# Maryamsana-1998/DiffCodec-Controlling-Latent-Diffusion-for-Perceptual-Video-Compression

Hardware: AMD Instinct MI355X
Metric: decoded frames/sec @ 512x512, 20-step DDIM, GOP-12 (higher is better)
Workload: dtype bf16; 1 GPU; 512x512 inter frames of a GOP-12 clip, 16 per step per GPU, 20-step DDIM, CFG 4.5 (model batch 32), control scale 1.7, SD-1.5 + DualFlowControlNet + VAE decode, random-init weights; hip_graphs=True, parallelism=unit-shard x1, backend=none, backend_world_size=1

## Files before the change

diffcodec-controlling-latent-diffusion-for-perceptual-video-compression_amd/csrc/attention.hip:

```cpp
#include "dc_common.h"
#include "../../include/diffcodec_hip.h"
#include <cstdlib>
#include <type_traits>

#ifdef DC_STAMP
__device__ unsigned long long dc_attn_stamp_buf[1 << 18];
extern "C" int dc_attn_stamp_read(void* dst, int n) { return (int)hipMemcpyFromSymbol(dst, HIP_SYMBOL(dc_attn_stamp_buf), (size_t)n * 8); }
#define DC_NOW(t) asm volatile("s_memtime %0\n\ts_waitcnt lgkmcnt(0)" : "=s"(t)::"memory")
#define DC_NOW_RT(t) asm volatile("s_memrealtime %0\n\ts_waitcnt lgkmcnt(0)" : "=s"(t)::"memory")
#define DC_STAMP_SLOTS 16
#else
#define DC_NOW(t) (void)0
#define DC_NOW_RT(t) (void)0
#endif

namespace {

constexpr int KV_TILE = 64;
constexpr float RESCALE_THR = 4.0f;
typedef __attribute__((ext_vector_type(4))) short s16x4;
typedef __attribute__((address_space(3))) s16x4* lds_s16x4_ptr;
__host__ __device__ constexpr int v_pitch_bytes(int ndt) { return ndt * 64 <= 64 ? 64 : (ndt * 64 <= 192 ? 192 : 320); }

struct AttnArgs {
    const bf16_t* q;
    const bf16_t* k;
    const bf16_t* v;
    bf16_t* o;
    int B, heads, Nq, Nk;
    long long qs, ks, vs, os;
    float scale_log2e;
    int xcd_remap;
};

constexpr int SHORT_PASSES = 4;
template <int D, int QB, bool SHORT, bool RAGGED, bool PP = false>
__global__ __launch_bounds__(PP ? 512 : 256, (D <= 80 ? 2 : 1)) void attn_kernel(const AttnArgs a)
{
    static_assert(!PP || !SHORT, "ping-pong is the long-context form");
    constexpr int NWAVE = PP ? 8 : 4, NT = NWAVE * 64;
    constexpr int ND16 = (D + 15) / 16;
    constexpr int NDT = (D + 31) / 32;
    constexpr int NV = D / 8;
    constexpr int KP16 = (ND16 * 2) | 1;
    constexpr int K_PITCH = KP16 * 16;
    constexpr int K_BYTES = KV_TILE * K_PITCH;
    constexpr int V_PITCH = v_pitch_bytes(NDT);
    constexpr int VT_BYTES = KV_TILE * V_PITCH;
    constexpr int BUF = K_BYTES + VT_BYTES;
    constexpr int QW = 32 * QB;
    constexpr int OPITCH = D * 2 + 16;
    static_assert(NDT <= 5, "head dim <= 160");
    constexpr bool QOFF = (D % 16) != 0 && !SHORT;
    constexpr int QOFF_KS = D / 16, QOFF_LH = (D % 16) / 8, QOFF_E = (D % 16) % 8;
    constexpr bool ONES = (D % 32) != 0;
    constexpr int ONES_T = D / 32, ONES_R = ((D % 32) & 3) + 4 * ((D % 32) >> 3);
    static_assert(!ONES || ((D % 32) % 8) < 4, "ones row must live in the lower lane half");
    constexpr int NLD = (KV_TILE * NV + 255) / 256;
    extern __shared__ __attribute__((aligned(16))) char smem[];

    const int tid = threadIdx.x, lane = tid & 63, wave = __builtin_amdgcn_readfirstlane(tid >> 6);
    const int lq = lane & 31, lh = lane >> 5;
    unsigned long long st_in = 0, rt_in = 0, rt_0 = 0, rt_e = 0, st_out = 0, rt_out = 0;
    DC_NOW(st_in);
    DC_NOW_RT(rt_in);
    constexpr int QWG = NWAVE * QW * (SHORT ? SHORT_PASSES : 1);
    const int qblocks = (a.Nq + QWG - 1) / QWG;
    int bid = blockIdx.x;
    if (a.xcd_remap) bid = dc_xcd_remap(bid, gridDim.x);
    const int bh = bid / qblocks;
    const int qb = bid - bh * qblocks;
    const int b = bh / a.heads, h = bh - b * a.heads;
    int q0 = qb * QWG + wave * QW;

    const bf16_t* __restrict__ Q = a.q + (long long)b * a.Nq * a.qs + h * D;
    const bf16_t* __restrict__ K = a.k + (long long)b * a.Nk * a.ks + h * D;
    const bf16_t* __restrict__ V = a.v + (long long)b * a.Nk * a.vs + h * D;

    for (int i = tid * 16; i < 2 * BUF; i += NT * 16) *(u32x4*)(smem + i) = u32x4{0u, 0u, 0u, 0u};
    if (ONES) {
        __syncthreads();
        if (tid < 2 * KV_TILE) {
            *(unsigned short*)(smem + (tid >> 6) * BUF + K_BYTES + (tid & 63) * V_PITCH + D * 2) = 0x3F80;
            if (QOFF) *(unsigned short*)(smem + (tid >> 6) * BUF + (tid & 63) * K_PITCH + D * 2) = 0x3F80;
        }
    }

    bf16x8 qf[QB][ND16];
    f32x16 oacc[QB][NDT];
    float m_run[QB], l_run[QB];
    auto fetch_q = [&](int qbase, bf16x8 (&dst)[QB][ND16]) {
#pragma unroll
        for (int u = 0; u < QB; ++u)
#pragma unroll
            for (int ks = 0; ks < ND16; ++ks) {
                const int dcol = 16 * ks + 8 * lh;
                const int qi = qbase + 32 * u + lq;
                u32x4 v = {0u, 0u, 0u, 0u};
                if (qi < a.Nq && dcol < D) v = *(const u32x4*)(Q + (long long)qi * a.qs + dcol);
                bf16x8 qv = *(bf16x8*)&v;
                if (QOFF) {
#pragma unroll
                    for (int e = 0; e < 8; ++e) qv[e] = (bf16_t)((float)qv[e] * a.scale_log2e);
                }
                dst[u][ks] = qv;
            }
    };
    auto reset_acc = [&]() {
#pragma unroll
        for (int u = 0; u < QB; ++u) {
#pragma unroll
            for (int t = 0; t < NDT; ++t)
#pragma unroll
                for (int r = 0; r < 16; ++r) oacc[u][t][r] = 0.f;
            m_run[u] = QOFF ? 0.f : -INFINITY;
            l_run[u] = 0.f;
        }
    };
    fetch_q(q0, qf);
    reset_acc();

    u32x4 rk[NLD], rv[NLD];
    const int ntiles = (a.Nk + KV_TILE - 1) / KV_TILE;

    constexpr int NVB = 4 * (NV / 4);
    auto v_piece = [&](int q, int& row, int& vec) {
        row = lane, vec = q;
        if (NVB > 0 && q < NVB) row = 16 * (q & 3) + (lane >> 2), vec = 4 * (q >> 2) + (lane & 3);
    };
    auto issue_loads = [&](int t) {
        const int kb = t * KV_TILE;
        int key = kb + lane;
        if (RAGGED) key = key < a.Nk ? key : a.Nk - 1;
#pragma unroll
        for (int i = 0; i < NLD; ++i) {
            const int vec = wave + 4 * i;
            if (vec < NV) {
                rk[i] = *(const u32x4*)(K + (long long)key * a.ks + vec * 8);
                int vrow, vvec;
                v_piece(vec, vrow, vvec);
                int vkey = kb + vrow;
                if (RAGGED) vkey = vkey < a.Nk ? vkey : a.Nk - 1;
                rv[i] = *(const u32x4*)(V + (long long)vkey * a.vs + vvec * 8);
            }
        }
    };
    auto store_lds = [&](int buf) {
        char* sK = smem + buf * BUF;
        char* sV = sK + K_BYTES;
#pragma unroll
        for (int i = 0; i < NLD; ++i) {
            const int vec = wave + 4 * i;
            if (vec < NV) {
                *(u32x4*)(sK + lane * K_PITCH + vec * 16) = rk[i];
                int vrow, vvec;
                v_piece(vec, vrow, vvec);
                *(u32x4*)(sV + vrow * V_PITCH + vvec * 16) = rv[i];
            }
        }
    };

    __syncthreads();
    if constexpr (!PP) {
        issue_loads(0);
        store_lds(0);
    }
    if constexpr (!PP) {
        __builtin_amdgcn_s_waitcnt(0x0F70);
        __syncthreads();
    }

    typedef __attribute__((ext_vector_type(2))) float f32x2;
    unsigned long long st_a = 0, st_b = 0, st_c = 0, st_d = 0, st_e = 0, s_qk = 0, s_sm = 0, s_pv = 0, s_st = 0, st_0 = 0, st_v = 0, s_vst = 0;
    DC_NOW(st_0);
    DC_NOW_RT(rt_0);
    f32x16 s[QB][2];
    bf16x8 pf[QB][2][2];
    int jn = 2;
    auto qk_part = [&](int buf) {
        const char* sK = smem + buf * BUF;
#pragma unroll
        for (int u = 0; u < QB; ++u)
#pragma unroll
            for (int j = 0; j < 2; ++j)
#pragma unroll
                for (int r = 0; r < 16; ++r) s[u][j][r] = 0.f;
#pragma unroll
        for (int j = 0; j < 2; ++j)
#pragma unroll
            for (int ks = 0; ks < ND16; ++ks) {
                if (j >= jn) continue;
                const bf16x8 kf = *(const bf16x8*)(sK + (32 * j + lq) * K_PITCH + (16 * ks + 8 * lh) * 2);
#pragma unroll
                for (int u = 0; u < QB; ++u) s[u][j] = __builtin_amdgcn_mfma_f32_32x32x16_bf16(kf, qf[u][ks], s[u][j], 0, 0, 0);
            }

    };
    float mloc_s[QB];
    auto rowmax_part = [&](int t) {
        const int kb = t * KV_TILE;
#pragma unroll
        for (int u = 0; u < QB; ++u) {
            if (RAGGED && kb + KV_TILE > a.Nk) {
#pragma unroll
                for (int j = 0; j < 2; ++j)
#pragma unroll
                    for (int r = 0; r < 16; ++r) {
                        if (j >= jn) continue;
                        const int key = kb + 32 * j + (r & 3) + 8 * (r >> 2) + 4 * lh;
                        if (key >= a.Nk) s[u][j][r] = -INFINITY;
                    }
            }
            float mloc = s[u][0][0];
#pragma unroll
            for (int j = 0; j < 2; ++j)
#pragma unroll
                for (int r = 0; r < 16; ++r)
                    if (j < jn) mloc = fmaxf(mloc, s[u][j][r]);
            {
                const auto sw = __builtin_amdgcn_permlane32_swap(__float_as_uint(mloc), __float_as_uint(mloc), false, false);
                mloc = fmaxf(__uint_as_float(sw[0]), __uint_as_float(sw[1]));
            }
            mloc_s[u] = mloc;
        }
    };
    auto softmax_part = [&](int t, bool first) {
        __builtin_amdgcn_s_setprio(2);
#pragma unroll
        for (int u = 0; u < QB; ++u) {
            const float mloc = mloc_s[u];
            if (QOFF) {
                const float m_next = (float)(bf16_t)(m_run[u] + mloc);
                const float delta = (first || mloc > RESCALE_THR) ? m_next - m_run[u] : 0.f;
                if (__any(delta != 0.f)) {
                    const float alpha = __builtin_amdgcn_exp2f(-delta);
#pragma unroll
                    for (int j = 0; j < 2; ++j)
#pragma unroll
                        for (int r = 0; r < 16; ++r) s[u][j][r] -= delta;
                    if (!ONES) l_run[u] *= alpha;
#pragma unroll
                    for (int tt = 0; tt < NDT; ++tt)
#pragma unroll
                        for (int r = 0; r < 16; ++r) oacc[u][tt][r] *= alpha;
                    m_run[u] += delta;
                    if (lh == QOFF_LH) qf[u][QOFF_KS][QOFF_E] = (bf16_t)(-m_run[u]);
                }
                float lsum = 0.f;
#pragma unroll
                for (int j = 0; j < 2; ++j)
#pragma unroll
                    for (int r = 0; r < 16; r += 2) {
                        const float p0 = __builtin_amdgcn_exp2f(s[u][j][r]), p1 = __builtin_amdgcn_exp2f(s[u][j][r + 1]);
                        if (!ONES) lsum += p0 + p1;
                        pf[u][j][r >> 3][r & 7] = (bf16_t)p0;
                        pf[u][j][r >> 3][(r & 7) + 1] = (bf16_t)p1;
                    }
                if (!ONES) l_run[u] += lsum;
                continue;
            }
            const float m_new = fmaxf(m_run[u], mloc);
            const float mc = m_new * a.scale_log2e;
            float lsum = 0.f;
#pragma unroll
            for (int j = 0; j < 2; ++j)
#pragma unroll
                for (int r = 0; r < 16; r += 2) {
                    if (j >= jn) continue;
                    const float t0 = __builtin_fmaf(s[u][j][r], a.scale_log2e, -mc), t1 = __builtin_fmaf(s[u][j][r + 1], a.scale_log2e, -mc);
                    const float p0 = __builtin_amdgcn_exp2f(t0), p1 = __builtin_amdgcn_exp2f(t1);
                    if (!ONES) lsum += p0 + p1;
                    pf[u][j][r >> 3][r & 7] = (bf16_t)p0;
                    pf[u][j][r >> 3][(r & 7) + 1] = (bf16_t)p1;
                }
            if (__any(m_new != m_run[u])) {
                const float alpha = __builtin_amdgcn_exp2f(m_run[u] * a.scale_log2e - mc);
                if (!ONES) l_run[u] *= alpha;
#pragma unroll
                for (int tt = 0; tt < NDT; ++tt)
#pragma unroll
                    for (int r = 0; r < 16; ++r) oacc[u][tt][r] *= alpha;
                m_run[u] = m_new;
            }
            if (!ONES) l_run[u] += lsum;
        }

        __builtin_amdgcn_s_setprio(0);
    };
    auto pv_part = [&](int buf) {
        const char* sV = smem + buf * BUF + K_BYTES;
        const char* vbase = sV + (4 * lh + ((lane & 15) >> 2)) * V_PITCH + (16 * ((lane >> 4) & 1) + 4 * (lane & 3)) * 2;
#pragma unroll
        for (int tt = 0; tt < NDT; ++tt) {
#pragma unroll
            for (int j = 0; j < 2; ++j)
#pragma unroll
                for (int s2 = 0; s2 < 2; ++s2) {
                    if (j >= jn) continue;
                    const char* pk = vbase + (32 * j + 16 * s2) * V_PITCH + tt * 64;
                    const s16x4 lo = __builtin_amdgcn_ds_read_tr16_b64_v4i16((lds_s16x4_ptr)pk);
                    const s16x4 hi = __builtin_amdgcn_ds_read_tr16_b64_v4i16((lds_s16x4_ptr)(pk + 8 * V_PITCH));
                    u32x2 l2 = *(const u32x2*)&lo, h2 = *(const u32x2*)&hi;
                    u32x4 av = {l2[0], l2[1], h2[0], h2[1]};
#pragma unroll
                    for (int u = 0; u < QB; ++u)
                        oacc[u][tt] = __builtin_amdgcn_mfma_f32_32x32x16_bf16(*(bf16x8*)&av, pf[u][j][s2], oacc[u][tt], 0, 0, 0);
                }
        }
    };
    auto process_tile = [&](int t, bool first, bool stage_next) {
        qk_part(t & 1);
        rowmax_part(t);
#ifdef DC_STAMP
        __builtin_amdgcn_sched_barrier(0);
        DC_NOW(st_b);
#endif
        softmax_part(t, first);
#ifdef DC_STAMP
        __builtin_amdgcn_sched_barrier(0);
        DC_NOW(st_c);
#endif
        if (stage_next) store_lds((t & 1) ^ 1);
        pv_part(t & 1);
    };

    auto store_out = [&]() {
#pragma unroll
    for (int u = 0; u < QB; ++u) {
        float l_tot;
        if (ONES) l_tot = __shfl(oacc[u][ONES_T][ONES_R], lq, 64);
        else l_tot = l_run[u] + __shfl_xor(l_run[u], 32, 64);
        const float inv = 1.0f / l_tot;
        const int qi = q0 + 32 * u + lq;
        if constexpr (SHORT) {
            char* stg = smem + 2 * BUF + wave * (QW * OPITCH) + (32 * u + lq) * OPITCH;
#pragma unroll
            for (int tt = 0; tt < NDT; ++tt)
#pragma unroll
                for (int g = 0; g < 4; ++g) {
                    const int dcol = 32 * tt + 8 * g + 4 * lh;
                    if (dcol < D) {
                        bf16x4 pk;
#pragma unroll
                        for (int r = 0; r < 4; ++r) pk[r] = (bf16_t)(oacc[u][tt][4 * g + r] * inv);
                        *(bf16x4*)(stg + dcol * 2) = pk;
                    }
                }
        } else if (qi < a.Nq) {
            bf16_t* __restrict__ O = a.o + ((long long)b * a.Nq + qi) * a.os + h * D;
#pragma unroll
            for (int tt = 0; tt < NDT; ++tt)
#pragma unroll
                for (int g = 0; g < 4; ++g) {
                    const int dcol = 32 * tt + 8 * g + 4 * lh;
                    if (dcol < D) {
                        bf16x4 pk;
#pragma unroll
                        for (int r = 0; r < 4; ++r) pk[r] = (bf16_t)(oacc[u][tt][4 * g + r] * inv);
                        *(bf16x4*)(O + dcol) = pk;
                    }
                }
        }
    }
    if constexpr (SHORT) {
        __builtin_amdgcn_fence(__ATOMIC_RELEASE, "wavefront");
        __builtin_amdgcn_wave_barrier();
        __builtin_amdgcn_fence(__ATOMIC_ACQUIRE, "wavefront");
        const char* stw = smem + 2 * BUF + wave * (QW * OPITCH);
        for (int i = lane; i < QW * NV; i += 64) {
            const int row = i / NV, pc = i - row * NV;
            const int qi = q0 + row;
            if (qi < a.Nq)
                *(u32x4*)(a.o + ((long long)b * a.Nq + qi) * a.os + h * D + pc * 8) = *(const u32x4*)(stw + row * OPITCH + pc * 16);
        }
        __builtin_amdgcn_fence(__ATOMIC_RELEASE, "wavefront");
        __builtin_amdgcn_wave_barrier();
    }
    };

    if constexpr (PP) {
        const int grp = wave >> 2, w4 = wave & 3;
        u32x4 rs[NLD];
        auto pp_piece = [&](int q, int& row, int& vec) {
            row = lane, vec = q;
            if (NVB > 0 && grp && q < NVB) row = 16 * (q & 3) + (lane >> 2), vec = 4 * (q >> 2) + (lane & 3);
        };
        auto pp_issue = [&](int t) {
#pragma unroll
            for (int i = 0; i < NLD; ++i) {
                const int q = w4 + 4 * i;
                if (q < NV) {
                    int row, vec;
                    pp_piece(q, row, vec);
                    int key = t * KV_TILE + row;
                    if (RAGGED) key = key < a.Nk ? key : a.Nk - 1;
                    const bf16_t* __restrict__ src = grp ? V + (long long)key * a.vs : K + (long long)key * a.ks;
                    rs[i] = *(const u32x4*)(src + vec * 8);
                }
            }
        };
        auto pp_store = [&](int buf) {
            char* base = smem + buf * BUF + (grp ? K_BYTES : 0);
            const int pitch = grp ? V_PITCH : K_PITCH;
#pragma unroll
            for (int i = 0; i < NLD; ++i) {
                const int q = w4 + 4 * i;
                if (q < NV) {
                    int row, vec;
                    pp_piece(q, row, vec);
                    *(u32x4*)(base + row * pitch + vec * 16) = rs[i];
                }
            }
        };
        const int T = ntiles;
        pp_issue(0);
        if (grp == 0) pp_store(0);
        __builtin_amdgcn_s_waitcnt(0x0F70);
        __syncthreads();
        if (grp == 1) __syncthreads();
        if (grp == 0 && 1 < T) pp_issue(1);
        qk_part(0);
        rowmax_part(0);
        if (grp == 1) pp_store(1);
        __syncthreads();
        if (grp == 1 && 1 < T) pp_issue(1);
        softmax_part(0, true);
        if (grp == 0 && 1 < T) pp_store(1);
        __syncthreads();
        for (int t = 1; t < T; ++t) {
            DC_NOW(st_a);
            if (grp == 0 && t + 1 < T) pp_issue(t + 1);
            qk_part(t & 1);
            pv_part(t & 1);
            rowmax_part(t);
            __builtin_amdgcn_sched_barrier(0);
#ifdef DC_STAMP
            DC_NOW(st_v);
#endif
            if (grp == 1) pp_store((t + 1) & 1);
#ifdef DC_STAMP
            __builtin_amdgcn_sched_barrier(0);
            DC_NOW(st_b);
            s_vst += st_b - st_v;
#endif
            __syncthreads();
            DC_NOW(st_c);
            if (grp == 1 && t + 1 < T) pp_issue(t + 1);
            softmax_part(t, false);
            __builtin_amdgcn_sched_barrier(0);
            if (grp == 0 && t + 1 < T) pp_store((t + 1) & 1);
#ifdef DC_STAMP
            __builtin_amdgcn_sched_barrier(0);
            DC_NOW(st_d);
#endif
            __syncthreads();
#ifdef DC_STAMP
            DC_NOW(st_e);
            s_qk += st_b - st_a, s_sm += st_c - st_b, s_pv += st_d - st_c, s_st += st_e - st_d;
#endif
        }
        pv_part(T & 1);
        if (grp == 0) __syncthreads();
#ifdef DC_STAMP
        DC_NOW(st_e);
        DC_NOW_RT(rt_e);
#endif
        store_out();
#ifdef DC_STAMP
        __builtin_amdgcn_s_waitcnt(0x0F70);
        DC_NOW(st_out);
        DC_NOW_RT(rt_out);
        if (lane == 0 && (long long)blockIdx.x * 8 + wave < (1 << 14)) {
            unsigned long long* o = dc_attn_stamp_buf + ((long long)blockIdx.x * 8 + wave) * DC_STAMP_SLOTS;
            o[0] = s_qk, o[1] = s_sm, o[2] = s_pv, o[3] = s_st, o[4] = st_e - st_0, o[5] = 1;
            o[6] = st_out - st_in, o[7] = rt_e - rt_0, o[8] = rt_in, o[9] = rt_out;
            o[10] = __builtin_amdgcn_s_getreg((31 << 11) | 4), o[11] = __builtin_amdgcn_s_getreg((31 << 11) | 20);
            o[12] = st_0 - st_in, o[13] = st_out - st_e;
            o[14] = s_vst;
        }
#endif
    } else if constexpr (!SHORT) {
        for (int t = 0; t < ntiles; ++t) {
            const bool more = t + 1 < ntiles;
            DC_NOW(st_a);
            if (more) issue_loads(t + 1);
            process_tile(t, t == 0, more);
#ifdef DC_STAMP
            __builtin_amdgcn_sched_barrier(0);
            DC_NOW(st_d);
#endif
            __syncthreads();
#ifdef DC_STAMP
            DC_NOW(st_e);
            s_qk += st_b - st_a, s_sm += st_c - st_b, s_pv += st_d - st_c, s_st += st_e - st_d;
#endif
        }
        store_out();
#ifdef DC_STAMP
        DC_NOW(st_e);
        if (lane == 0) {
            unsigned long long* o = dc_attn_stamp_buf + ((long long)blockIdx.x * 4 + wave) * DC_STAMP_SLOTS;
            if ((long long)blockIdx.x * 4 + wave < (1 << 14)) o[0] = s_qk, o[1] = s_sm, o[2] = s_pv, o[3] = s_st, o[4] = st_e - st_0;
        }
#endif
    } else {
        if (ntiles > 1) {
            issue_loads(1);
            store_lds(1);
            __syncthreads();
        }
        for (int pass = 0;; ++pass) {
            const bool has_next = pass + 1 < SHORT_PASSES && q0 + 4 * QW < a.Nq;
            bf16x8 qn[QB][ND16];
            if (has_next) fetch_q(q0 + 4 * QW, qn);
            for (int t = 0; t < ntiles; ++t) {
                jn = (t * KV_TILE + 32 >= a.Nk) ? 1 : 2;
                process_tile(t, t == 0, false);
            }
            store_out();
            if (!has_next) break;
            q0 += 4 * QW;
#pragma unroll
            for (int u = 0; u < QB; ++u)
#pragma unroll
                for (int ks = 0; ks < ND16; ++ks) qf[u][ks] = qn[u][ks];
            reset_acc();
        }
    }
}

template <int D, int QB, bool SHORT, bool RAGGED, bool PP = false>
int launch_qb_r(const AttnArgs& a, hipStream_t st)
{
    constexpr int ND16 = (D + 15) / 16, NDT = (D + 31) / 32;
    constexpr int KP16 = (ND16 * 2) | 1;
    constexpr int BUF = KV_TILE * KP16 * 16 + KV_TILE * v_pitch_bytes(NDT);
    const size_t lds = 2 * BUF + (SHORT ? 4 * (32 * QB) * (D * 2 + 16) : 0);
    auto kern = attn_kernel<D, QB, SHORT, RAGGED, PP>;
    static std::atomic<unsigned long long> attr_done{0};
    dc_set_max_dyn_lds((const void*)kern, (int)lds, attr_done);
    constexpr int QWG = (PP ? 256 : 128) * QB * (SHORT ? SHORT_PASSES : 1);
    const int qblocks = (a.Nq + QWG - 1) / QWG;
    hipLaunchKernelGGL(kern, dim3(a.B * a.heads * qblocks), dim3(PP ? 512 : 256), lds, st, a);
    return dc_launch_status();
}

struct AttnForm {
    int qb;
    bool shrt, ragged, pp;
};

AttnForm attn_form(int D, int B, int heads, int Nq, int Nk)
{
    const bool short_ctx = Nk <= 2 * KV_TILE;
    const bool ragged = (Nk % KV_TILE) != 0;
    if (D <= 48) {
        const long long wgs2 = (long long)B * heads * ((Nq + 255) / 256);
        if (wgs2 >= 512) {
            if (short_ctx && (long long)B * heads * ((Nq + 127) / 128) / SHORT_PASSES >= 512) return {1, true, true, false};
            if (short_ctx && wgs2 / SHORT_PASSES >= 512) return {2, true, true, false};
            const long long wgs_pp = (long long)B * heads * ((Nq + 511) / 512);
            if (!short_ctx && wgs_pp >= 256 && Nk >= 4 * KV_TILE) return {2, false, ragged, true};
            return {2, false, ragged, false};
        }
    }
    const long long wgs1 = (long long)B * heads * ((Nq + 127) / 128);
    if (short_ctx && wgs1 / SHORT_PASSES >= 512) return {1, true, true, false};
    return {1, false, ragged, false};
}

template <int D>
int launch(const AttnArgs& a, hipStream_t st)
{
    const AttnForm f = attn_form(D, a.B, a.heads, a.Nq, a.Nk);
    if constexpr (D <= 48) {
        if (f.qb == 2) {
            if (f.pp) return f.ragged ? launch_qb_r<D, 2, false, true, true>(a, st) : launch_qb_r<D, 2, false, false, true>(a, st);
            if (f.shrt) return launch_qb_r<D, 2, true, true>(a, st);
            return f.ragged ? launch_qb_r<D, 2, false, true>(a, st) : launch_qb_r<D, 2, false, false>(a, st);
        }
    }
    if (f.shrt) return launch_qb_r<D, 1, true, true>(a, st);
    return f.ragged ? launch_qb_r<D, 1, false, true>(a, st) : launch_qb_r<D, 1, false, false>(a, st);
}

template <class F>
int with_head_dim(int D, F&& f)
{
    switch (D) {
        case 8: return f(std::integral_constant<int, 8>{});
        case 16: return f(std::integral_constant<int, 16>{});
        case 32: return f(std::integral_constant<int, 32>{});
        case 40: return f(std::integral_constant<int, 40>{});
        case 64: return f(std::integral_constant<int, 64>{});
        case 80: return f(std::integral_constant<int, 80>{});
        case 128: return f(std::integral_constant<int, 128>{});
        case 160: return f(std::integral_constant<int, 160>{});
        default: return DC_ERR_INVALID;
    }
}

__global__ __launch_bounds__(256) void softmax_rows_kernel(const float* __restrict__ s, bf16_t* __restrict__ p,
                                                            int cols, float scale)
{
    __shared__ float red[8];
    const long long row = blockIdx.x;
    const float* x = s + row * cols;
    float m = -INFINITY;
    for (int i = threadIdx.x; i < cols; i += 256) m = fmaxf(m, x[i] * scale);
    m = dc_wave_max(m);
    if ((threadIdx.x & 63) == 0) red[threadIdx.x >> 6] = m;
    __syncthreads();
    m = fmaxf(fmaxf(red[0], red[1]), fmaxf(red[2], red[3]));
    float sum = 0.f;
    for (int i = threadIdx.x; i < cols; i += 256) sum += __expf(x[i] * scale - m);
    sum = dc_wave_sum(sum);
    if ((threadIdx.x & 63) == 0) red[4 + (threadIdx.x >> 6)] = sum;
    __syncthreads();
    const float inv = 1.0f / (red[4] + red[5] + red[6] + red[7]);
    bf16_t* o = p + row * cols;
    for (int i = threadIdx.x; i < cols; i += 256) o[i] = (bf16_t)(__expf(x[i] * scale - m) * inv);
}

}

extern "C" int dc_attention_bf16(const void* q, const void* k, const void* v, void* out, int B, int heads, int Nq,
                                 int Nk, int D, long long q_stride, long long k_stride, long long v_stride,
                                 long long o_stride, float scale, void* stream)
{
    if (!q || !k || !v || !out || B <= 0 || heads <= 0 || Nq <= 0 || Nk <= 0) return DC_ERR_INVALID;
    if ((q_stride | k_stride | v_stride | o_stride) & 7) return DC_ERR_INVALID;
    AttnArgs a{(const bf16_t*)q, (const bf16_t*)k, (const bf16_t*)v, (bf16_t*)out, B, heads, Nq, Nk,
               q_stride, k_stride, v_stride, o_stride, scale * 1.4426950408889634f, 1};
    hipStream_t st = (hipStream_t)stream;
    return with_head_dim(D, [&](auto dc) { return launch<decltype(dc)::value>(a, st); });
}

extern "C" int dc_attention_route(int B, int heads, int Nq, int Nk, int D, int* info)
{
    if (!info) return DC_ERR_INVALID;
    for (int i = 0; i < DC_ATTN_ROUTE_INFO_INTS; ++i) info[i] = 0;
    if (B <= 0 || heads <= 0 || Nq <= 0 || Nk <= 0) return DC_ERR_INVALID;
    if (with_head_dim(D, [](auto) { return (int)DC_OK; }) != DC_OK) return DC_ERR_INVALID;
    const AttnForm f = attn_form(D, B, heads, Nq, Nk);
    info[0] = D;
    info[1] = f.qb;
    info[2] = f.shrt;
    info[3] = f.ragged;
    info[4] = f.pp;
    return DC_OK;
}

extern "C" int dc_softmax_rows_f32_to_bf16(const float* s, void* p, long long rows, int cols, float scale, void* stream)
{
    if (!s || !p || rows <= 0 || cols <= 0) return DC_ERR_INVALID;
    hipLaunchKernelGGL(softmax_rows_kernel, dim3((unsigned)rows), dim3(256), 0, (hipStream_t)stream, s, (bf16_t*)p, cols, scale);
    return dc_launch_status();
}
```

Measured before the change: 20.04 frames/s.

## Specialize short-KV attention path by key-tile count with single-shot softmax

```diff
diff --git a/diffcodec-controlling-latent-diffusion-for-perceptual-video-compression_amd/csrc/attention.hip b/diffcodec-controlling-latent-diffusion-for-perceptual-video-compression_amd/csrc/attention.hip
--- a/diffcodec-controlling-latent-diffusion-for-perceptual-video-compression_amd/csrc/attention.hip
+++ b/diffcodec-controlling-latent-diffusion-for-perceptual-video-compression_amd/csrc/attention.hip
@@ -324,7 +324,7 @@
         pv_part(t & 1);
     };
 
-    auto store_out = [&]() {
+    auto store_out = [&](auto tail_rows) {
 #pragma unroll
     for (int u = 0; u < QB; ++u) {
         float l_tot;
@@ -367,11 +367,22 @@
         __builtin_amdgcn_wave_barrier();
         __builtin_amdgcn_fence(__ATOMIC_ACQUIRE, "wavefront");
         const char* stw = smem + 2 * BUF + wave * (QW * OPITCH);
-        for (int i = lane; i < QW * NV; i += 64) {
+        bf16_t* __restrict__ ob = a.o + ((long long)b * a.Nq + q0) * a.os + h * D;
+        constexpr int NP = QW * NV, NFULL = NP / 64;
+        static_assert(NP % 64 == 0 || NP % 64 == 32, "whole or half waves of pieces");
+        constexpr bool TAIL = decltype(tail_rows)::value;
+#pragma unroll
+        for (int it = 0; it < NFULL; ++it) {
+            const int i = lane + 64 * it;
             const int row = i / NV, pc = i - row * NV;
-            const int qi = q0 + row;
-            if (qi < a.Nq)
-                *(u32x4*)(a.o + ((long long)b * a.Nq + qi) * a.os + h * D + pc * 8) = *(const u32x4*)(stw + row * OPITCH + pc * 16);
+            if (!TAIL || q0 + row < a.Nq)
+                *(u32x4*)(ob + (long long)row * a.os + pc * 8) = *(const u32x4*)(stw + row * OPITCH + pc * 16);
+        }
+        if constexpr (NP % 64 != 0) {
+            const int i = 64 * NFULL + (lane >> 1);
+            const int row = i / NV, pc = i - row * NV;
+            if (!TAIL || q0 + row < a.Nq)
+                *(u32x2*)(ob + (long long)row * a.os + pc * 8 + 4 * (lane & 1)) = *(const u32x2*)(stw + row * OPITCH + pc * 16 + 8 * (lane & 1));
         }
         __builtin_amdgcn_fence(__ATOMIC_RELEASE, "wavefront");
         __builtin_amdgcn_wave_barrier();
@@ -465,7 +476,7 @@
         DC_NOW(st_e);
         DC_NOW_RT(rt_e);
 #endif
-        store_out();
+        store_out(std::false_type{});
 #ifdef DC_STAMP
         __builtin_amdgcn_s_waitcnt(0x0F70);
         DC_NOW(st_out);
@@ -495,7 +506,7 @@
             s_qk += st_b - st_a, s_sm += st_c - st_b, s_pv += st_d - st_c, s_st += st_e - st_d;
 #endif
         }
-        store_out();
+        store_out(std::false_type{});
 #ifdef DC_STAMP
         DC_NOW(st_e);
         if (lane == 0) {
@@ -509,22 +520,139 @@
             store_lds(1);
             __syncthreads();
         }
-        for (int pass = 0;; ++pass) {
-            const bool has_next = pass + 1 < SHORT_PASSES && q0 + 4 * QW < a.Nq;
-            bf16x8 qn[QB][ND16];
-            if (has_next) fetch_q(q0 + 4 * QW, qn);
-            for (int t = 0; t < ntiles; ++t) {
-                jn = (t * KV_TILE + 32 >= a.Nk) ? 1 : 2;
-                process_tile(t, t == 0, false);
-            }
-            store_out();
-            if (!has_next) break;
-            q0 += 4 * QW;
-#pragma unroll
-            for (int u = 0; u < QB; ++u)
-#pragma unroll
-                for (int ks = 0; ks < ND16; ++ks) qf[u][ks] = qn[u][ks];
-            reset_acc();
+        auto short_passes = [&](auto nhc, auto tailc) {
+            constexpr int NH = decltype(nhc)::value;
+            constexpr bool TAIL = decltype(tailc)::value;
+            constexpr int NH0 = NH < 2 ? NH : 2;
+            const int lim = a.Nk - 32 * (NH - 1) - 4 * lh;
+            const char* kb0 = smem + lq * K_PITCH + 16 * lh;
+            const char* vb0 = smem + K_BYTES + (4 * lh + ((lane & 15) >> 2)) * V_PITCH + (16 * ((lane >> 4) & 1) + 4 * (lane & 3)) * 2;
+            constexpr bool QPART = (D % 16) != 0;
+            auto fetch = [&](int qbase, bf16x8 (&dst)[QB][ND16]) {
+#pragma unroll
+                for (int u = 0; u < QB; ++u) {
+                    const int qi = min(qbase + 32 * u + lq, a.Nq - 1);
+                    const bf16_t* __restrict__ qp = Q + (long long)qi * a.qs;
+#pragma unroll
+                    for (int ks = 0; ks < ND16; ++ks) {
+                        const u32x4 v = *(const u32x4*)(qp + 16 * ks + ((QPART && ks == ND16 - 1) ? 0 : 8 * lh));
+                        dst[u][ks] = *(const bf16x8*)&v;
+                    }
+                }
+            };
+            auto one_pass = [&](bf16x8 (&qc)[QB][ND16], bool more) {
+                f32x16 sh[QB][NH];
+                bf16x8 ph[QB][NH][2];
+                bf16x8 qlast[QB];
+#pragma unroll
+                for (int u = 0; u < QB; ++u) {
+                    u32x4 v = *(const u32x4*)&qc[u][ND16 - 1];
+                    if (QPART && lh) v = u32x4{0u, 0u, 0u, 0u};
+                    qlast[u] = *(const bf16x8*)&v;
+                }
+#pragma unroll
+                for (int hh = 0; hh < NH; ++hh)
+#pragma unroll
+                    for (int ks = 0; ks < ND16; ++ks) {
+                        const bf16x8 kf = *(const bf16x8*)(kb0 + (hh >> 1) * BUF + (hh & 1) * 32 * K_PITCH + 32 * ks);
+#pragma unroll
+                        for (int u = 0; u < QB; ++u) {
+                            f32x16 c = {0.f, 0.f, 0.f, 0.f, 0.f, 0.f, 0.f, 0.f, 0.f, 0.f, 0.f, 0.f, 0.f, 0.f, 0.f, 0.f};
+                            if (ks) c = sh[u][hh];
+                            sh[u][hh] = __builtin_amdgcn_mfma_f32_32x32x16_bf16(kf, ks == ND16 - 1 ? qlast[u] : qc[u][ks], c, 0, 0, 0);
+                        }
+                    }
+                if (more) fetch(q0 + 4 * QW, qc);
+                float m0[QB], m1[QB];
+#pragma unroll
+                for (int u = 0; u < QB; ++u) {
+#pragma unroll
+                    for (int r = 0; r < 16; ++r)
+                        if ((r & 3) + 8 * (r >> 2) >= lim) sh[u][NH - 1][r] = -INFINITY;
+                    auto row_max = [&](int h0, int h1) {
+                        float m = sh[u][h0][0];
+#pragma unroll
+                        for (int hh = h0; hh < h1; ++hh)
+#pragma unroll
+                            for (int r = 0; r < 16; ++r) m = fmaxf(m, sh[u][hh][r]);
+                        const auto sw = __builtin_amdgcn_permlane32_swap(__float_as_uint(m), __float_as_uint(m), false, false);
+                        return fmaxf(__uint_as_float(sw[0]), __uint_as_float(sw[1]));
+                    };
+                    m0[u] = row_max(0, NH0);
+                    m1[u] = m0[u];
+                    if constexpr (NH > 2) m1[u] = fmaxf(m0[u], row_max(2, NH));
+                    const float mc0 = m0[u] * a.scale_log2e, mc1 = m1[u] * a.scale_log2e;
+                    float ls[2] = {0.f, 0.f};
+                    __builtin_amdgcn_s_setprio(2);
+#pragma unroll
+                    for (int hh = 0; hh < NH; ++hh)
+#pragma unroll
+                        for (int r = 0; r < 16; r += 2) {
+                            const float mc = hh < 2 ? mc0 : mc1;
+                            const float t0 = __builtin_fmaf(sh[u][hh][r], a.scale_log2e, -mc), t1 = __builtin_fmaf(sh[u][hh][r + 1], a.scale_log2e, -mc);
+                            const float p0 = __builtin_amdgcn_exp2f(t0), p1 = __builtin_amdgcn_exp2f(t1);
+                            if (!ONES) ls[hh >> 1] += p0 + p1;
+                            ph[u][hh][r >> 3][r & 7] = (bf16_t)p0;
+                            ph[u][hh][r >> 3][(r & 7) + 1] = (bf16_t)p1;
+                        }
+                    __builtin_amdgcn_s_setprio(0);
+                    l_run[u] = ls[0];
+                    if constexpr (NH > 2) {
+                        if (__any(m1[u] != m0[u])) l_run[u] *= __builtin_amdgcn_exp2f(__builtin_fmaf(m0[u], a.scale_log2e, -mc1));
+                        l_run[u] += ls[1];
+                    }
+                }
+                auto pv = [&](int h0, int h1) {
+#pragma unroll
+                    for (int tt = 0; tt < NDT; ++tt)
+#pragma unroll
+                        for (int hh = h0; hh < h1; ++hh)
+#pragma unroll
+                            for (int s2 = 0; s2 < 2; ++s2) {
+                                const char* pk = vb0 + (hh >> 1) * BUF + (32 * (hh & 1) + 16 * s2) * V_PITCH + tt * 64;
+                                const s16x4 lo = __builtin_amdgcn_ds_read_tr16_b64_v4i16((lds_s16x4_ptr)pk);
+                                const s16x4 hi = __builtin_amdgcn_ds_read_tr16_b64_v4i16((lds_s16x4_ptr)(pk + 8 * V_PITCH));
+                                u32x2 l2 = *(const u32x2*)&lo, h2 = *(const u32x2*)&hi;
+                                u32x4 av = {l2[0], l2[1], h2[0], h2[1]};
+#pragma unroll
+                                for (int u = 0; u < QB; ++u) {
+                                    f32x16 c = {0.f, 0.f, 0.f, 0.f, 0.f, 0.f, 0.f, 0.f, 0.f, 0.f, 0.f, 0.f, 0.f, 0.f, 0.f, 0.f};
+                                    if (hh | s2) c = oacc[u][tt];
+                                    oacc[u][tt] = __builtin_amdgcn_mfma_f32_32x32x16_bf16(*(bf16x8*)&av, ph[u][hh][s2], c, 0, 0, 0);
+                                }
+                            }
+                };
+                pv(0, NH0);
+                if constexpr (NH > 2) {
+#pragma unroll
+                    for (int u = 0; u < QB; ++u)
+                        if (__any(m1[u] != m0[u])) {
+                            const float alpha = __builtin_amdgcn_exp2f(__builtin_fmaf(m0[u], a.scale_log2e, -m1[u] * a.scale_log2e));
+#pragma unroll
+                            for (int tt = 0; tt < NDT; ++tt)
+#pragma unroll
+                                for (int r = 0; r < 16; ++r) oacc[u][tt][r] *= alpha;
+                        }
+                    pv(2, NH);
+                }
+                store_out(tailc);
+            };
+            for (int pass = 0;; ++pass) {
+                const bool more = pass + 1 < SHORT_PASSES && (!TAIL || q0 + 4 * QW < a.Nq);
+                one_pass(qf, more);
+                if (!more) break;
+                q0 += 4 * QW;
+            }
+        };
+        auto with_tail = [&](auto nhc) {
+            if (qb * QWG + QWG <= a.Nq) short_passes(nhc, std::false_type{});
+            else short_passes(nhc, std::true_type{});
+        };
+        switch ((a.Nk + 31) >> 5) {
+            case 1: with_tail(std::integral_constant<int, 1>{}); break;
+            case 2: with_tail(std::integral_constant<int, 2>{}); break;
+            case 3: with_tail(std::integral_constant<int, 3>{}); break;
+            default: with_tail(std::integral_constant<int, 4>{}); break;
         }
     }
 }
```

After: 20.10 frames/s (median of 6 runs). No clear change (+0.3%).
